# ipfs/go-libp2p-pubsub

Hardware: AMD Instinct MI355X
Metric: deliveries/sec (peer×msg) at 1M peers, 1/2/4/8 GPU; % of HBM roofline (higher is better)
Workload: dtype u64

## Files before the change

go-libp2p-pubsub_amd/csrc/api.cpp:

```cpp
#include <algorithm>
#include <cstdio>
#include <cstdlib>
#include <cstring>

#include "engine.hpp"
#include "psengine_plan.h"

using namespace psamd;

namespace {

TopicHost* join_topic(ps_engine* e, uint32_t topic) {
  if (!topic_ok(e, topic)) {
    e->fail(PS_E_STATE, "no such topic");
    return nullptr;
  }
  TopicHost& T = e->topics[topic];
  if (T.kind != Kind::Join) {
    e->fail(PS_E_STATE, "topic topology was set explicitly");
    return nullptr;
  }
  return &T;
}

// ... 99 lines not shown
  g_abi_error = buf;
  return PS_E_INVAL;
}

static bool env_flag(const char* name, bool cur) {
  const char* v = std::getenv(name);
  return v ? std::atoi(v) != 0 : cur;
}
static uint32_t env_u32(const char* name, int lo, int hi, uint32_t cur) {
  const char* v = std::getenv(name);
  return v ? static_cast<uint32_t>(std::min(hi, std::max(lo, std::atoi(v)))) : cur;
}
static uint64_t env_u64(const char* name, int base, uint64_t cur) {
  const char* v = std::getenv(name);
  return v ? std::strtoull(v, nullptr, base) : cur;
}

static void read_switches(ps_engine* e) {
  constexpr int kAny = 0x7FFFFFFF;
  auto& s = e->env;
  auto& d = e->drain.env;
  s.host_timing = env_flag("PSAMD_HOST_TIMING", s.host_timing);
  s.flood_profile = env_flag("PSAMD_FLOOD_PROFILE", s.flood_profile);
  if (const char* v = std::getenv("PSAMD_CHAIN_PROFILE")) s.chain_prof_path = v;
  d.timing = env_flag("PSAMD_DRAIN_TIMING", d.timing);
  if (!env_flag("PSAMD_AB", false)) return;
  d.slab_ids = std::max<uint64_t>(kDrainSegBits, env_u64("PSAMD_DRAIN_SLAB_IDS", 10, d.slab_ids));
  if (const char* v = std::getenv("PSAMD_DRAIN_EMIT")) d.staged = std::strcmp(v, "direct") != 0;
  if (const char* v = std::getenv("PSAMD_DRAIN_ASYNC_OUT")) d.mapped_out = std::strcmp(v, "mapped") == 0;
  if (const char* v = std::getenv("PSAMD_DRAIN_SHARED")) d.share = std::strcmp(v, "private") != 0;
  if (const char* v = std::getenv("PSAMD_LOAD_COUNT")) d.load_rows = std::strcmp(v, "rows") == 0;
  s.twin = env_flag("PSAMD_TWIN", s.twin);
  s.expand_opts = env_flag("PSAMD_NARROW", true) ? 0u : kExpandNoNarrow;
  s.chain_words_lead = env_u32("PSAMD_CHAIN_WORDS_LEAD", 0, 1 << 20, s.chain_words_lead);
  s.upload_reuse = env_flag("PSAMD_UPLOAD_REUSE", s.upload_reuse);
  s.sig_windows = env_flag("PSAMD_SIG_WINDOWS", s.sig_windows);
  s.fuse_reduce = env_flag("PSAMD_FUSE_REDUCE", s.fuse_reduce);
  ps_plan_opts o = e->opts;
  o.gpu_build = env_flag("PSAMD_GPU_BUILD", o.gpu_build);
  o.flood = env_flag("PSAMD_FLOOD", o.flood);
  if (!env_flag("PSAMD_PULL_PAIR", true)) o.chain_max = o.chain_max_groups = 1;
  if (const char* v = std::getenv("PSAMD_XCHG_OVERLAP")) o.xchg_overlap = std::atoi(v) != 0;
  o.chain_max = env_u32("PSAMD_CHAIN", 1, kChainLevels, o.chain_max);
  o.chain_max_groups = env_u32("PSAMD_CHAIN", 1, kChainLevels, o.chain_max_groups);
  o.overlap = env_flag("PSAMD_OVERLAP", o.overlap);
  o.overlap_min_rounds = env_u32("PSAMD_OVERLAP_ROUNDS", 2, kAny, o.overlap_min_rounds);
  o.overlap_min_bytes = env_u64("PSAMD_OVERLAP_BYTES", 10, o.overlap_min_bytes);
  o.pad_words = env_u32("PSAMD_PAD_WORDS", 2, kAny, o.pad_words);
  o.chain_tail = env_flag("PSAMD_CHAIN_TAIL", o.chain_tail);
  if (const char* v = std::getenv("PSAMD_LAUNCH_BYTES"))
    o.launch_bytes = static_cast<uint64_t>(std::max(0.0, std::atof(v)));
  o.chain_words = env_u32("PSAMD_CHAIN_WORDS", 256, 1 << 20, o.chain_words);
  o.flood_words = env_u32("PSAMD_FLOOD_WORDS", 64, 1 << 16, o.flood_words);
  o.flood_spin_ticks = static_cast<uint32_t>(env_u64("PSAMD_FLOOD_SPIN_TICKS", 0, o.flood_spin_ticks));
  o.flood_top_bytes = env_u64("PSAMD_FLOOD_TOP_BYTES", 0, o.flood_top_bytes);
  o.flood_min_rounds = env_u32("PSAMD_FLOOD_MIN_ROUNDS", 1, kAny, o.flood_min_rounds);
  o.chain_waves = env_u32("PSAMD_CHAIN_WAVES", 0, 16, o.chain_waves);
  if (!check_opts(o)) e->opts = o;
}

int ps_plan_opts_default(ps_plan_opts* out) {
  if (!out) return PS_E_INVAL;
  *out = default_plan_opts();
  return PS_OK;
}

// ... 861 lines not shown
```

go-libp2p-pubsub_amd/csrc/engine.hpp:

```cpp
#pragma once
#include <hip/hip_runtime.h>

#include <chrono>
#include <cstdlib>
#include <cstdint>
#include <map>
#include <memory>
#include <string>
#include <utility>
#include <vector>

#include "dist.hpp"
#include "kernels.hpp"
#include "psengine.h"
#include "tree.hpp"

namespace psamd {

constexpr uint32_t kMaxRoundsCap = 4096;
constexpr uint32_t kAlignedRowsMax = 2 * (PS_MAX_ROUNDS + 1);
constexpr uint32_t kMaxStartRound = 200;
constexpr uint32_t kDefaultWindow = 65536;
constexpr uint32_t kMaxWindow = 1u << 30;

// ... 767 lines not shown
  return t < e->last_pos.size() && !e->last_pos[t].empty() ? e->last_pos[t].data() : nullptr;
}
inline uint32_t window_bit(const uint32_t* bits, uint32_t li) { return bits ? bits[li] : li; }
inline const std::vector<uint32_t>& peer_node_map(ps_engine* e, uint32_t topic, const TopicDev& d) {
  auto& pm = e->peer_node[topic];
  if (e->peer_node_epoch.size() != e->topics.size()) e->peer_node_epoch.assign(e->topics.size(), ~0ull);
  if (e->peer_node_epoch[topic] != e->graph_epoch) {
    pm.assign(e->cfg.n_peers, kNone);
    const uint32_t u0 = (d.flags & kTopicRootLocal) ? 1 : 0;
    for (uint32_t k = u0; k < d.n_nodes; ++k) pm[e->node_peer[d.nbase + k]] = k;
    e->peer_node_epoch[topic] = e->graph_epoch;
  }
  return pm;
}

int plan_window_layout(ps_engine* e, const std::vector<RunMsg>& msgs, const std::vector<WinSlice>& win,
                       WindowLayout& L);
bool plan_pull_chunks(ps_engine* e, const WindowLayout& L);
bool plan_pair_chunks(ps_engine* e, const WindowLayout& L, uint32_t first);
bool plan_flood_tasks(ps_engine* e, const WindowLayout& L, uint32_t rounds);
int plan_ghost(ps_engine* e, const WindowLayout& L, bool* changed);
void annotate_chunks(ps_engine* e, const WindowLayout& L);
uint32_t plan_flood_rounds(const ps_engine* e, const WindowLayout& L);
bool deep_window(const ps_engine* e, const WindowLayout& L);
int plan_window_schedule(ps_engine* e, const std::vector<RunMsg>& msgs, const std::vector<WinSlice>& win,
                         WindowLayout& L, WindowSchedule& S);
void plan_schedule_pairs(ps_engine* e, const WindowLayout& L, WindowSchedule& S);
uint32_t round_grid(const ps_engine* e, const WindowLayout& L, const WindowSchedule& S, uint32_t r);

int run_body(ps_engine* e, ps_stats* st, bool may_defer);
bool accumulate_window(ps_stats* st, const uint64_t* hs, const uint64_t* ha, uint32_t r, uint32_t planned0,
                       uint32_t mode, uint32_t flood_rounds, uint32_t launches, int32_t world,
                       const std::vector<uint8_t>& kinds, bool by_round = true);
bool split_aligned_window(ps_stats* st, const uint64_t* hs, uint32_t r, uint32_t true_rounds,
                          const AlignedSplit& sp, std::string* why = nullptr);

}
```

go-libp2p-pubsub_amd/csrc/kernels.hip:

```cpp
#include <algorithm>

#include "devutil.hpp"
#include "kernels.hpp"

namespace psamd {

namespace {

using namespace dev;

__device__ __forceinline__ uint32_t wave_incl_scan(uint32_t v) {
  const int lane = threadIdx.x & 63;
#pragma unroll
  for (int d = 1; d < 64; d <<= 1) {
    uint32_t t = __shfl_up(v, d, 64);
    if (lane >= d) v += t;
  }
  return v;
}

__device__ __forceinline__ uint32_t block_excl_scan(uint32_t v, uint32_t* total) {
  __shared__ uint32_t wsum[kBlock / 64];
  const int lane = threadIdx.x & 63, wid = threadIdx.x >> 6;
  uint32_t inc = wave_incl_scan(v);
// ... 223 lines not shown
        const int q = __ffsll(static_cast<long long>(b)) - 1;
        rec[q] = hop_round(round);
        b &= b - 1;
      }
    }
  }
}

__device__ __forceinline__ void mark_next(const ExpandArgs& a, uint32_t c) {
  a.next_flag[c] = 1;
  a.blk_flag[c >> kFlagBlockShift] = 1;
}

__device__ __forceinline__ uint32_t rl(uint32_t v, uint32_t lane) {
  return static_cast<uint32_t>(__builtin_amdgcn_readlane(static_cast<int>(v), static_cast<int>(lane)));
}

__device__ __forceinline__ uint32_t pow2_shift(uint32_t W) { return 32u - __clz(W - 1u); }

#define PSAMD_LDS_DMA(g, lds_base, N)                                            \
  __builtin_amdgcn_global_load_lds((const __attribute__((address_space(1))) void*)(g), \
                                   (__attribute__((address_space(3))) void*)(lds_base), N, 0, 0)

constexpr uint32_t kStageWords = 704;
constexpr uint32_t kStageBytes = 512;
struct __attribute__((aligned(16))) WaveStage {
  uint64_t words[kStageWords];
  uint8_t flags[kStageBytes];
  uint8_t gens[kStageBytes];
};

struct EntryCtr {
  uint32_t ent = 0, ent_words = 0, kids = 0, mesh_kids = 0, clear = 0;
};

__device__ __forceinline__ bool ext_rows(const ExpandArgs& a, uint32_t W, uint32_t tflags) {
  return a.ext_cur != nullptr && W >= 64 && W <= kStageWords && !(tflags & (kTopicSingleStart | kTopicMesh));
}
constexpr uint32_t ext_whole(uint32_t W) { return W << 16; }
__device__ __forceinline__ uint32_t ext_of(const ExpandArgs& a, uint32_t p, uint32_t W) {
  const uint32_t x = a.ext_cur[p];
  return (x >> 16) <= W && (x & 0xFFFFu) <= (x >> 16) ? x : ext_whole(W);
}

template <bool kRecord>
__device__ void expand_direct(const ExpandArgs& a, uint32_t p, uint32_t rs, uint32_t deg,
                              uint32_t c0, uint32_t W, uint32_t nbase, uint32_t tflags,
                              uint64_t wbase, uint32_t lane, uint32_t cur, uint32_t round,
                              ExpandCtr& k, EntryCtr& ec) {
  const bool mesh = (tflags & kTopicMesh) != 0;
  const bool split = (tflags & kEntrySplit) != 0;
  const bool listed = mesh || split;
  const bool is_root = p == nbase && (tflags & kTopicRootLocal);
  const bool single = (tflags & kTopicSingleStart) && !mesh;
  const uint64_t* src = (single && !is_root) ? a.seen : a.a_cur;
  const uint64_t pw = wbase + static_cast<uint64_t>(p - nbase) * W;
  const uint64_t cbase = wbase - static_cast<uint64_t>(nbase) * W;
  const bool ext = ext_rows(a, W, tflags);
  const uint32_t xe = ext && !is_root ? ext_of(a, p, W) : ext_whole(W);
  const uint32_t xlo = xe & 0xFFFFu, xhi = xe >> 16;
  ec.ent += 1;
  ec.ent_words += W;
  ec.kids += deg;
  if (mesh) ec.mesh_kids += deg;
  for (uint32_t j0 = 0; j0 < deg; j0 += 64) {
    const uint32_t cd = min(64u, deg - j0);
    uint32_t cj = 0, fj = 0, gj = 0;
    if (lane < cd) {
      cj = listed ? a.col[rs + j0 + lane] : c0 + j0 + lane;
      if (!(cj & kRemoteBit)) {
        fj = a.node_flags[cj];
        gj = mesh ? 0u : a.gen[cj];
      }
    }
    if (split) {
      for (uint32_t jj = 0; jj < cd; ++jj) {
        const uint32_t c = rl(cj, jj);
        if (!(c & kRemoteBit)) continue;
        const uint32_t dest = (c >> kRemoteRankShift) & 0xFu;
        uint8_t* region = a.send + a.send_off[dest];
        uint32_t base = 0;
        if (lane == 0) base = atomicAdd(reinterpret_cast<uint32_t*>(region), W);
        base = static_cast<uint32_t>(__shfl(static_cast<int>(base), 0, 64));
        XItem* out = reinterpret_cast<XItem*>(region + kRegionHeader) + base;
        for (uint32_t w = lane; w < W; w += 64) {
          XItem it;
          it.node = c & kRemoteIdMask;
          it.word = w;
          it.mask = src[pw + w];
          out[w] = it;
        }
      }
    }
    if (W >= 64) {
      for (uint32_t wb = 0; wb < W; wb += 64) {
        const uint32_t w = wb + lane;
        const bool active = w < W;
        const uint64_t m = active && w >= xlo && w < xhi ? src[pw + w] : 0ull;
        for (uint32_t jj = 0; jj < cd; ++jj) {
          const uint32_t f = rl(fj, jj);
          if (!(f & kNodeLive)) continue;
          const uint32_t c = rl(cj, jj);
          const bool stale = !mesh && rl(gj, jj) != cur;
          const bool internal = (f & kNodeInternal) != 0;
          uint64_t nm = 0;
          if (active)
            nm = deliver_word<kRecord>(a, mesh, stale, internal && !single,
                                       cbase + static_cast<uint64_t>(c) * W + w, m, round, k);
          if (internal && __ballot(nm != 0) && lane == 0) {
            mark_next(a, c);
            if (ext) a.ext_next[c] = xe;
          }
        }
      }
    } else {
      const uint32_t sh = pow2_shift(W);
      const uint32_t wp = 1u << sh;
      const uint32_t w = lane & (wp - 1u);
      const uint32_t jl = lane >> sh;
      const uint32_t groups = 64u >> sh;
      const uint64_t gmask = (wp == 64u ? ~0ull : ((1ull << wp) - 1ull)) << (jl << sh);
      const uint64_t m = w < W ? src[pw + w] : 0ull;
      for (uint32_t jb = 0; jb < cd; jb += groups) {
        const uint32_t jj = jb + jl;
        const uint32_t c = static_cast<uint32_t>(__shfl(static_cast<int>(cj), static_cast<int>(jj), 64));
        const uint32_t f = static_cast<uint32_t>(__shfl(static_cast<int>(fj), static_cast<int>(jj), 64));
        const uint32_t g = static_cast<uint32_t>(__shfl(static_cast<int>(gj), static_cast<int>(jj), 64));
        const bool live = (w < W) && (jj < cd) && (f & kNodeLive);
        uint64_t nm = 0;
        if (live)
          nm = deliver_word<kRecord>(a, mesh, !mesh && g != cur,
                                     (f & kNodeInternal) != 0 && !single,
                                     cbase + static_cast<uint64_t>(c) * W + w, m, round, k);
        const uint64_t bal = __ballot(nm != 0);
        if (live && w == 0 && (f & kNodeInternal) && (bal & gmask)) mark_next(a, c);
      }
    }
    if (!mesh && lane < cd && (fj & kNodeLive))
      a.gen[cj] = static_cast<uint8_t>(cur);
  }
  if (mesh || is_root) {
    for (uint32_t w = lane; w < W; w += 64) a.a_cur[pw + w] = 0;
    ec.clear += W;
  }
}

template <bool kRecord>
__device__ void expand_wide(const ExpandArgs& a, WaveStage& ws, uint32_t p, uint32_t deg,
                            uint32_t c0, uint32_t W, uint32_t nbase, uint32_t fl, uint64_t wbase,
                            uint32_t lane, uint32_t cur, uint32_t round, ExpandCtr& k,
                            EntryCtr& ec) {
  const bool is_root = p == nbase && (fl & kTopicRootLocal);
  const bool from_seen = (fl & kTopicSingleStart) && !is_root;
  const bool keep = !(fl & kTopicSingleStart);
  const uint64_t pw = wbase + static_cast<uint64_t>(p - nbase) * W;
  const uint64_t cbase = wbase - static_cast<uint64_t>(nbase) * W;
  const uint32_t* row = reinterpret_cast<const uint32_t*>((from_seen ? a.seen : a.a_cur) + pw);
  uint32_t fj = 0, gj = 0;
  if (lane < deg) {
    fj = a.node_flags[c0 + lane];
    gj = a.gen[c0 + lane];
  }
  ec.ent += 1;
  ec.ent_words += W;
  ec.kids += deg;
  uint64_t got = 0;
  for (uint32_t w0 = 0; w0 < W; w0 += kStageWords) {
    const uint32_t len = min(kStageWords, W - w0);
// ... 217 lines not shown
        if (e.xe) a.ext_next[c] = e.xe;
      }
    }
  }
  ec.ent += static_cast<uint32_t>(__popcll(fmask));
  ec.ent_words += static_cast<uint32_t>(wave_sum_u64(L));
  ec.kids += ktotal;
  return flat;
}

template <bool kRecord, bool kDirect>
__global__ __launch_bounds__(kBlock) __attribute__((amdgpu_waves_per_eu(6))) void k_expand(ExpandArgs a,
                                                                                            uint32_t round) {
  __shared__ WaveStage stage_lds[kDirect ? 1 : kBlock / 64];
  const uint32_t lane = threadIdx.x & 63;
  const uint32_t wave =
      __builtin_amdgcn_readfirstlane((blockIdx.x * kBlock + threadIdx.x) >> 6);
  WaveStage& ws = stage_lds[kDirect ? 0 : __builtin_amdgcn_readfirstlane(threadIdx.x >> 6)];
  const uint32_t n_waves = (gridDim.x * kBlock) >> 6;
  const uint32_t n = *a.n_front;
  const uint32_t cur = a.gen_cur & 0xFF;

  ExpandCtr k;
  EntryCtr ec;

  const uint32_t v = __builtin_amdgcn_readfirstlane(
      (gridDim.x & 7u) ? wave
                       : ((blockIdx.x & 7u) * (gridDim.x >> 3) + (blockIdx.x >> 3)) * (kBlock / 64) +
                             (threadIdx.x >> 6));
  for (uint64_t e0 = v; e0 < n; e0 += 64ull * n_waves) {
    const uint64_t el = e0 + static_cast<uint64_t>(lane) * n_waves;
    uint32_t bp = 0, brs = 0, bdeg = 0, bc0 = 0, bW = 0, bnb = 0, bfl = 0, bwl = 0, bwh = 0, bex = 0;
    uint32_t brl = 0, brh = 0, bcl = 0, bch = 0, bnd = 0, bst = 0;
    if (el < n) {
      bp = a.frontier[el];
      const uint32_t t = a.node_topic[bp];
      brs = a.row_ptr[bp];
      bdeg = a.row_ptr[bp + 1] - brs;
      const TopicDev T = a.topics[t];
      bW = T.W;
      bnb = T.nbase;
      bfl = T.flags | ((a.node_flags[bp] & kNodeSplit) ? kEntrySplit : 0u);
      bwl = static_cast<uint32_t>(T.wbase);
      bwh = static_cast<uint32_t>(T.wbase >> 32);
      if (bdeg && T.W) bc0 = a.col[brs];
      bex = ext_rows(a, T.W, T.flags) && !(bp == T.nbase && (T.flags & kTopicRootLocal)) ? ext_of(a, bp, T.W)
                                                                                          : ext_whole(T.W);
    }
    const uint32_t nb = static_cast<uint32_t>(__popcll(__ballot(el < n)));
    const bool is_root = bp == bnb && (bfl & kTopicRootLocal);
    const bool staged = el < n && bW > 0 && !(bfl & (kTopicMesh | kEntrySplit)) && bW <= kStageWords && bdeg <= 64;
    if constexpr (!kRecord && !kDirect) {
      if (flat_on(a)) {
        const bool short_row = staged && !is_root && (bex >> 16) - (bex & 0xFFFFu) < kFlatWords;
        const uint64_t wbase = (static_cast<uint64_t>(bwh) << 32) | bwl;
        const uint64_t src = reinterpret_cast<uint64_t>(((bfl & kTopicSingleStart) ? a.seen : a.a_cur) + wbase +
                                                        static_cast<uint64_t>(bp - bnb) * bW + (bex & 0xFFFFu));
        const uint64_t crow = wbase + static_cast<uint64_t>(bc0 - bnb) * bW;
        if (expand_flat(a, ws, short_row, bW, bex, short_row && ext_rows(a, bW, bfl), bdeg, bc0, src, crow,
                        !(bfl & kTopicSingleStart), lane, cur, k, ec))
          bW = 0;
      }
    }
    if (el < n && bW) {
      const uint64_t wbase = (static_cast<uint64_t>(bwh) << 32) | bwl;
      const bool from_seen = (bfl & kTopicSingleStart) && !is_root;
      const uint64_t rp = reinterpret_cast<uint64_t>((from_seen ? a.seen : a.a_cur) + wbase +
                                                     static_cast<uint64_t>(bp - bnb) * bW + (bex & 0xFFFFu));
      brl = static_cast<uint32_t>(rp);
      brh = static_cast<uint32_t>(rp >> 32);
      const uint64_t cb = wbase + static_cast<uint64_t>(bc0 - bnb) * bW;
      bcl = static_cast<uint32_t>(cb);
      bch = static_cast<uint32_t>(cb >> 32);
      bnd = ((bc0 + bdeg + 3u) >> 2) - (bc0 >> 2);
      const uint32_t Ls = (bex >> 16) - (bex & 0xFFFFu);
      bst = staged ? (Ls + (Ls & 1u)) | (4u * bnd) << 16 : ~0u;
    }
    uint32_t q = 0;
    while (q < nb) {
      const uint32_t W0 = rl(bW, q), d0 = rl(bdeg, q), f0 = rl(bfl, q);
      if (W0 == 0) {
        ++q;
        continue;
      }
      const bool direct = (f0 & (kTopicMesh | kEntrySplit)) || d0 > 64;
      if (direct || kDirect) {
        if (direct && kDirect)
          expand_direct<kRecord>(a, rl(bp, q), rl(brs, q), d0, rl(bc0, q), W0, rl(bnb, q), f0,
                                 (static_cast<uint64_t>(rl(bwh, q)) << 32) | rl(bwl, q), lane,
                                 cur, round, k, ec);
        ++q;
        continue;
      }
      if (W0 > kStageWords) {
        expand_wide<kRecord>(a, ws, rl(bp, q), d0, rl(bc0, q), W0, rl(bnb, q), f0,
                                     (static_cast<uint64_t>(rl(bwh, q)) << 32) | rl(bwl, q), lane,
                                     cur, round, k, ec);
        ++q;
        continue;
// ... 16 lines not shown
          const uint32_t c0 = rl(bc0, i);
          const uint32_t xe = rl(bex, i), lo = xe & 0xFFFFu, L = (xe >> 16) - lo;
          const uint32_t* row =
              reinterpret_cast<const uint32_t*>((static_cast<uint64_t>(rl(brh, i)) << 32) | rl(brl, i));
          uint32_t* dst = reinterpret_cast<uint32_t*>(ws.words + off);
          if ((W & 1u) == 0) {
            for (uint32_t d = 0; d < 2 * L; d += 256)
              if (d + 4 * lane < 2 * L) PSAMD_LDS_DMA(row + d + 4 * lane, dst + d, 16);
          } else {
            for (uint32_t d = 0; d < 2 * L; d += 64)
              if (d + lane < 2 * L) PSAMD_LDS_DMA(row + d + lane, dst + d, 4);
          }
          const uint32_t nd = rl(bnd, i);
          if (lane < nd) {
            PSAMD_LDS_DMA(reinterpret_cast<const uint32_t*>(a.node_flags) + (c0 >> 2) + lane,
                          ws.flags + doff, 4);
            PSAMD_LDS_DMA(reinterpret_cast<const uint32_t*>(a.gen) + (c0 >> 2) + lane,
                          ws.gens + doff, 4);
          }
          off += L + (L & 1u);
          doff += 4u * nd;
        }
        asm volatile("s_waitcnt vmcnt(0)" ::: "memory");
      }
      {
        uint32_t off = 0, doff = 0;
        for (uint32_t i = q; i < q + nq; ++i) {
          const uint32_t W = rl(bW, i), deg = rl(bdeg, i);
          if (W == 0) continue;
          const uint32_t c0 = rl(bc0, i);
          const uint64_t crow0 = (static_cast<uint64_t>(rl(bch, i)) << 32) | rl(bcl, i);
          const uint32_t nd = rl(bnd, i);
          const uint32_t fo = doff + (c0 & 3u);
          const bool keep = !(rl(bfl, i) & kTopicSingleStart);
          const uint32_t xe = rl(bex, i), lo = xe & 0xFFFFu, hi = xe >> 16;
          ec.ent += 1;
          ec.ent_words += hi - lo;
          ec.kids += deg;
          if (W >= 64) {
            const bool ext = ext_rows(a, W, rl(bfl, i));
            uint32_t tlo = lo, thi = hi;
            if (ext) {
              tlo = hi;
              thi = lo;
              for (uint32_t wb = lo; wb < hi; wb += 64) {
                const uint32_t w = wb + lane;
                const uint64_t nz = __ballot(w < hi && ws.words[off + w - lo] != 0);
                if (nz) {
                  tlo = min(tlo, wb + static_cast<uint32_t>(__ffsll(static_cast<long long>(nz))) - 1u);
                  thi = wb + 64u - static_cast<uint32_t>(__clzll(static_cast<long long>(nz)));
                }
              }
              if (tlo >= thi) {
                tlo = thi = lo;
              } else {
                tlo &= ~1u;
                thi = (thi + 1u) & ~1u;
              }
            }
            for (uint32_t jj = 0; jj < deg; ++jj) {
              const uint32_t f = ws.flags[fo + jj];
              if (!(f & kNodeLive)) continue;
              const bool stale = ws.gens[fo + jj] != cur;
              const bool internal = (f & kNodeInternal) != 0;
              const bool store = internal && keep;
              const uint32_t c = c0 + jj;
              const uint64_t row = crow0 + static_cast<uint64_t>(jj) * W;
              bool any = false;
              if (stale) {
                for (uint32_t wb = 0; wb < W; wb += 128) {
                  const uint32_t w = wb + 2 * lane;
                  if (w < W) {
                    const bool in = w >= tlo && w < thi;
                    const uint4 v = in ? *reinterpret_cast<const uint4*>(ws.words + off + w - lo)
                                       : make_uint4(0u, 0u, 0u, 0u);
                    deliver_fresh2<kRecord>(a, store && (in || !ext), row + w, v, round, k);
                    any |= (v.x | v.y | v.z | v.w) != 0;
                  }
                }
              } else {
                for (uint32_t wb = tlo; wb < thi; wb += 64) {
                  const uint32_t w = wb + lane;
                  if (w < thi) {
                    const uint64_t nm = deliver_tree<kRecord>(a, store, row + w, ws.words[off + w - lo], round, k);
                    any |= nm != 0;
                  }
                }
              }
              if (internal && __ballot(any) && lane == 0) {
                mark_next(a, c);
                if (ext) a.ext_next[c] = tlo | thi << 16;
              }
            }
          } else {
            const uint32_t sh = pow2_shift(W);
            const uint32_t wp = 1u << sh;
            const uint32_t w = lane & (wp - 1u);
            const uint32_t jl = lane >> sh;
            const uint32_t groups = 64u >> sh;
            const uint64_t gmask = (wp == 64u ? ~0ull : ((1ull << wp) - 1ull)) << (jl << sh);
            const uint64_t m = w < W ? ws.words[off + w] : 0ull;
            for (uint32_t jb = 0; jb < deg; jb += groups) {
              const uint32_t jj = jb + jl;
              const bool valid = (w < W) && (jj < deg);
              const uint32_t f = valid ? ws.flags[fo + jj] : 0u;
              const bool live = valid && (f & kNodeLive);
              const bool stale = ws.gens[fo + jj] != cur;
              const uint32_t c = c0 + jj;
              const uint64_t cw = crow0 + static_cast<uint64_t>(jj) * W + w;
              uint64_t nm = 0;
              if (__ballot(live && !stale) == 0) {
                if (live) {
                  deliver_fresh<kRecord>(a, keep && (f & kNodeInternal), cw, m, round, k);
                  nm = m;
                }
              } else if (live) {
                if (stale) {
                  deliver_fresh<kRecord>(a, keep && (f & kNodeInternal), cw, m, round, k);
                  nm = m;
                } else {
                  nm = deliver_tree<kRecord>(a, keep && (f & kNodeInternal), cw, m, round, k);
                }
              }
              const uint64_t bal = __ballot(nm != 0);
              if (live && w == 0 && (f & kNodeInternal) && (bal & gmask)) mark_next(a, c);
            }
          }
          if (lane < deg && (ws.flags[fo + lane] & kNodeLive))
            a.gen[c0 + lane] = static_cast<uint8_t>(cur);
          if (rl(bp, i) == rl(bnb, i) && (rl(bfl, i) & kTopicRootLocal)) {
            const uint64_t pw = (static_cast<uint64_t>(rl(bwh, i)) << 32) | rl(bwl, i);
            for (uint32_t w = lane; w < W; w += 64) a.a_cur[pw + w] = 0;
            ec.clear += W;
          }
          off += (hi - lo) + ((hi - lo) & 1u);
          doff += 4u * nd;
        }
      }
      q += nq;
    }
  }

  const uint64_t s_deliv = wave_sum_u64(k.deliv);
  const uint64_t s_dup = wave_sum_u64(k.dup);
  const uint64_t s_sr = wave_sum_u64(k.sr);
  const uint64_t s_sw = wave_sum_u64(k.sw);
  const uint64_t s_aw = wave_sum_u64(k.aw);
  if (lane == 0) {
    uint64_t* out = a.partials + static_cast<uint64_t>(wave) * kNumCtr;
    out[kCtrDeliveries] = s_deliv;
    out[kCtrDuplicates] = s_dup;
    out[kCtrEntries] = ec.ent;
    out[kCtrEntryWords] = ec.ent_words;
    out[kCtrChildren] = ec.kids;
    out[kCtrMeshChildren] = ec.mesh_kids;
    out[kCtrSeenReads] = s_sr;
    out[kCtrSeenWrites] = s_sw;
    out[kCtrArrivalWrites] = s_aw;
    out[kCtrClearWords] = ec.clear;
  }
}

__global__ __launch_bounds__(kBlock) void k_stage_copy(StageCopy c) {
  const uint32_t tid = blockIdx.x * kBlock + threadIdx.x, nth = gridDim.x * kBlock;
  for (uint32_t k = 0; k < c.n; ++k)
    for (uint32_t i = tid; i < c.words[k]; i += nth) c.dst[k][i] = c.src[k][i];
}

template <bool kRecord>
__global__ __launch_bounds__(kBlock) void k_apply(ApplyArgs a, uint32_t round) {
  const uint64_t total = a.cap_pre[a.world];
  uint64_t deliv = 0, dup = 0;
  for (uint64_t i = static_cast<uint64_t>(blockIdx.x) * kBlock + threadIdx.x; i < total;
       i += static_cast<uint64_t>(gridDim.x) * kBlock) {
    uint32_t src = 0;
    while (i >= a.cap_pre[src + 1]) ++src;
    const uint8_t* region = a.recv + a.recv_off[src];
    const uint64_t k = i - a.cap_pre[src];
    if (k >= *reinterpret_cast<const uint32_t*>(region)) continue;
    const XItem it = reinterpret_cast<const XItem*>(region + kRegionHeader)[k];
    const uint8_t f = a.node_flags[it.node];
    if (!(f & kNodeLive) || it.mask == 0) {
      if ((f & kNodeLive) && (f & kNodeInternal)) {
        const TopicDev T = a.topics[a.node_topic[it.node]];
        if (!(T.flags & kTopicSingleStart))
// ... 479 lines not shown
```

go-libp2p-pubsub_amd/csrc/kernels.hpp:

```cpp
#pragma once
#include <hip/hip_runtime.h>

#include <cstdint>

namespace psamd {

enum : uint8_t {
  kNodeLive = 1,
  kNodeInternal = 2,
  kNodeSplit = 4,
};

constexpr uint32_t kRemoteBit = 0x80000000u;
constexpr uint32_t kRemoteRankShift = 27;
constexpr uint32_t kRemoteIdMask = (1u << kRemoteRankShift) - 1u;
constexpr int kMaxRanks = 16;

struct XItem {
  uint32_t node;
  uint32_t word;
  uint64_t mask;
};
constexpr uint32_t kRegionHeader = 16;

// ... 43 lines not shown
  kCtrChildren,
  kCtrMeshChildren,
  kCtrSeenReads,
  kCtrSeenWrites,
  kCtrArrivalWrites,
  kCtrClearWords,
  kNumCtr
};

struct ExpandArgs {
  const uint32_t* frontier;
  const uint32_t* n_front;
  const uint32_t* row_ptr;
  const uint32_t* col;
  const uint16_t* node_topic;
  const uint8_t* node_flags;
  const TopicDev* topics;
  uint64_t* a_cur;
  uint64_t* a_next;
  uint64_t* seen;
  uint32_t* ext_cur;
  uint32_t* ext_next;
  uint8_t* gen;
  uint8_t* next_flag;
  uint8_t* blk_flag;
  uint64_t* partials;
  uint16_t* hop_rec;
  uint32_t gen_cur;
  uint8_t* send;
  uint64_t send_off[kMaxRanks];
  uint32_t opts;
};
constexpr uint32_t kExpandNoNarrow = 1;

struct PullChunk {
  uint32_t node_begin, node_end;
  uint32_t topic;
  uint32_t p_lo, p_hi;
  uint32_t W;
  uint32_t row0_lo, row0_hi;
  uint32_t e_lo, e_hi;
  uint32_t c_lo, c_hi;
  uint32_t gin, gout;
  uint32_t group;
  uint32_t lvl0;
};
constexpr uint32_t kPullMaxKids = 512;
constexpr uint32_t kNoneNode = 0xFFFFFFFFu;
constexpr uint32_t kPullWords = 1024;

struct ShipEntry {
  uint32_t node;
  uint32_t dst;
};
struct GhostSeg {
  uint64_t rbase[kMaxRanks];
  uint64_t sbase[kMaxRanks];
  uint32_t rw;
  uint32_t topic;
  uint32_t flags;
  uint32_t gbase[kMaxRanks];
};
constexpr uint32_t kSegInPlace = 1u;
struct RankRows {
  const uint64_t* seen;
  const uint8_t* gen;
// ... 670 lines not shown
```

go-libp2p-pubsub_amd/csrc/run.cpp:

```cpp
#include <algorithm>
#include <chrono>
#include <atomic>
#include <cstdio>
#include <cstdlib>
#include <cstring>
#include <thread>

#include "engine.hpp"
#include "gbuild.hpp"

namespace {
inline void cpu_relax() {
#if defined(__x86_64__) || defined(__i386__)
  __builtin_ia32_pause();
#else
  std::this_thread::yield();
#endif
}
}

namespace psamd {

namespace {

// ... 962 lines not shown
    std::string xerr;
    hipError_t xe =
        e->transport->exchange(a.send, s_off, s_len, e->d_recv.as<uint8_t>(), r_off, r_len, s, &xerr);
    if (xe != hipSuccess) return e->fail(PS_E_DEVICE, xerr);
    st->xchg_path = PS_XCHG_COPY;
    st->xchg_rounds += 1;
    for (const uint64_t n : r_len) st->xchg_bytes += n;
    HIP_TRY(launch_apply(apply_args(rr), rr, record, s), "apply");
    return PS_OK;
  }

  int grow_stats_rows(uint32_t planned) {
    const uint32_t rows = std::min<uint32_t>(L.round_cap, std::max(planned + 1, 2 * stats_rows));
    DevBuf grown;
    HIP_TRY(grown.ensure(static_cast<size_t>(rows + 1) * kNumCtr * 8), "grow stats");
    HIP_TRY(hipMemcpyAsync(grown.p, e->d_stats.p, static_cast<size_t>(stats_rows + 1) * kNumCtr * 8,
                           hipMemcpyDeviceToDevice, s),
            "keep stats");
    HIP_TRY(hipStreamSynchronize(s), "sync");
    std::swap(grown.p, e->d_stats.p);
    std::swap(grown.bytes, e->d_stats.bytes);
    stats = e->d_stats.as<uint64_t>();
    stats_rows = rows;
    return PS_OK;
  }

  int compaction_rounds() {
    const int32_t world = e->world;
    uint32_t planned = L.planned0;
    if (world > 1)
      for (auto* v : {&s_off, &s_len, &r_off, &r_len}) v->assign(world, 0);
    uint32_t* ext[2] = {nullptr, nullptr};
    if (world == 1) {
      HIP_TRY(e->d_ext0.ensure(static_cast<size_t>(e->n_pad) * 4), "alloc extents");
      HIP_TRY(e->d_ext1.ensure(static_cast<size_t>(e->n_pad) * 4), "alloc extents");
      ext[0] = e->d_ext0.as<uint32_t>();
      ext[1] = e->d_ext1.as<uint32_t>();
    }
    HIP_TRY(seed_round(0, arr[0]), "seed");
    HIP_TRY(compact_frontier(0, 0), "compact");
    while (true) {
      for (; r < planned && r < L.round_cap;) {
        ++r;
        a.a_cur = arr[(r - 1) & 1];
        a.a_next = arr[r & 1];
        a.ext_cur = ext[(r - 1) & 1];
        a.ext_next = ext[r & 1];
        const bool xr = layout_regions(r);
        if (xr)
          for (int32_t q = 0; q < world; ++q)
            if (s_len[q]) HIP_TRY(hipMemsetAsync(a.send + s_off[q], 0, kRegionHeader, s), "reset header");
        HIP_TRY(time_mark(true), "event");
        ++launches;
        const uint32_t grid_r = r <= L.planned0 ? round_grid(e, L, S, r) : e->expand_grid;
        a.partials = partials;
        HIP_TRY(launch_expand(a, r, record, grid_r, s), "expand");
        uint32_t waves_r = grid_r * (kBlock / 64);
        if (L.need_direct) {
          a.partials = partials + static_cast<size_t>(waves_r) * kNumCtr;
          HIP_TRY(launch_expand_direct(a, r, record, e->expand_grid, s), "expand direct");
          waves_r += n_waves;
        }
        HIP_TRY(time_mark(false), "event");
        if (xr)
          if (const int rc = exchange_apply(r)) return rc;
        HIP_TRY(seed_round(r, a.a_next), "seed");
        HIP_TRY(compact_frontier(r, waves_r), "compact");
      }
// ... 93 lines not shown
        }
      }
    }
    return PS_OK;
  }

  int finish_blocking() {
    const uint32_t planned0 = L.planned0;
    HIP_TRY(hipEventSynchronize(e->ev_run1), "sync");
    const auto t_sync = Clock::now();
    const ps_stats keep = *st;
    float ms = 0.f;
    HIP_TRY(hipEventElapsedTime(&ms, e->ev_run0, e->ev_run1), "elapsed");
    st->run_ms += ms;
    for (size_t i = 0; i < ev_used; i += 2) {
      float k = 0.f;
      HIP_TRY(hipEventElapsedTime(&k, e->ev_k[i], e->ev_k[i + 1]), "elapsed");
      st->expand_ms += k;
      const size_t q = ev_round[i / 2];
      if (q < PS_MAX_ROUNDS) st->expand_ms_per_round[q] += k;
    }
    std::vector<uint64_t> hs(static_cast<size_t>(r + 1 + S.reach_rows) * kNumCtr), ha;
    HIP_TRY(hipMemcpyAsync(hs.data(), stats, hs.size() * 8, hipMemcpyDeviceToHost, s), "read stats");
    if (e->world > 1) {
      ha.resize(static_cast<size_t>(planned0 + 1) * kNumCtr);
      HIP_TRY(hipMemcpyAsync(ha.data(), e->d_apply_stats.p, ha.size() * 8, hipMemcpyDeviceToHost, s),
              "read apply stats");
    }
    HIP_TRY(hipStreamSynchronize(s), "sync");
    if (S.mode == PS_MODE_FLOOD && e->env.flood_profile && e->flood_prof_waves) flood_profile_report(e);
    if (cprof) chain_profile_dump(e, planned0);
    if (std::string why; L.aligned && !split_aligned_window(st, hs.data(), r, L.true_rounds, L.split, &why))
      return e->fail(PS_E_DEVICE, "level-aligned window: reach counts disagree with the per-level counters (" + why + ")");
    if (!accumulate_window(st, hs.data(), ha.data(), r, planned0, S.mode, S.flood_rounds, launches, e->world,
                           e->round_kind, !L.aligned)) {
      e->flood_broken = true;
      *st = keep;
      if (e->env.host_timing) std::fprintf(stderr, "[psengine] k_flood timed out: window re-run per round\n");
      return run_window(e, msgs, win, st);
    }
    if (e->env.host_timing) {
      char tail[80];
      std::snprintf(tail, sizeof tail, ", wait %.3f ms, tail %.3f ms",
                    std::chrono::duration<double, std::milli>(t_sync - t_enq).count(),
                    std::chrono::duration<double, std::milli>(Clock::now() - t_sync).count());
      host_timing_line("window", tail);
    }
    if (record)
      if (const int rc = read_hop_record()) return rc;
    remember_window();
    return PS_OK;
  }

  int run() {
    int rc;
    if ((rc = window_layout())) return rc;
    if (L.wtot == 0 && e->world == 1) return PS_OK;
    t_w1 = Clock::now();
    if ((rc = ensure_window_buffers())) return rc;
    if ((rc = plan_window_schedule(e, msgs, win, L, S))) return rc;
    if ((rc = upload_window_plans()) || (rc = ensure_schedule_buffers())) return rc;
    t_w3 = Clock::now();
    if ((rc = upload_reach_pieces())) return rc;
    if ((rc = choose_streams()) || (rc = start_window())) return rc;
    if ((rc = L.level ? level_rounds() : compaction_rounds())) return rc;
    const bool defer = defers(r);
// ... 2 lines not shown
    t_enq = Clock::now();
    return defer ? finish_deferred() : finish_blocking();
  }
};

int run_window(ps_engine* e, const std::vector<RunMsg>& msgs, const std::vector<WinSlice>& win, ps_stats* st) {
  return WindowRun{e, msgs, win, st}.run();
}

int run_phase(ps_engine* e, const std::vector<RunMsg>& msgs, const std::vector<WinSlice>& per, ps_stats* st) {
  const uint32_t nt = static_cast<uint32_t>(e->topics.size());
  const uint32_t cap = e->cfg.msg_window;
  uint32_t n_win = 0;
  for (const auto& v : per) n_win = std::max(n_win, (v.n + cap - 1) / cap);
  std::vector<WinSlice> win(nt);
  for (uint32_t k = 0; k < n_win; ++k) {
    for (uint32_t t = 0; t < nt; ++t) {
      const uint32_t lo = k * cap;
      win[t].idx = per[t].idx + std::min(lo, per[t].n);
      win[t].n = lo < per[t].n ? std::min(cap, per[t].n - lo) : 0;
    }
    e->defer_last = e->defer_phase && k + 1 == n_win;
    const uint64_t seq0 = e->window_seq;
    int rc = run_window(e, msgs, win, st);
    e->defer_last = false;
    if (!rc && e->window_seq != seq0 && !(rc = sink_window(e)) && !(rc = load_window(e)) && !(rc = hops_window(e)) &&
        !(rc = downstream_window(e)) && !(rc = cut_window(e)))
      rc = report_window(e);
    if (rc) return rc;
  }
  return PS_OK;
}

}

bool accumulate_window(ps_stats* st, const uint64_t* hs, const uint64_t* ha, uint32_t r, uint32_t planned0,
                       uint32_t mode, uint32_t flood_rounds, uint32_t launches, int32_t world,
                       const std::vector<uint8_t>& kinds, bool by_round) {
  const bool pull = mode == PS_MODE_LEVEL_PULL || mode == PS_MODE_FLOOD;
  std::memset(st->round_kernel, 0, sizeof(st->round_kernel));
  for (uint32_t q = 1; q <= r; ++q) {
    const uint8_t kind = q < kinds.size() ? kinds[q] : static_cast<uint8_t>(pull ? PS_K_PULL : PS_K_EXPAND);
    const uint64_t* c = &hs[static_cast<size_t>(q) * kNumCtr];
    const uint64_t app_d = (world > 1 && q <= planned0) ? ha[static_cast<size_t>(q) * kNumCtr + kCtrDeliveries] : 0;
    const uint64_t app_u = (world > 1 && q <= planned0) ? ha[static_cast<size_t>(q) * kNumCtr + kCtrDuplicates] : 0;
    st->deliveries += c[kCtrDeliveries] + app_d;
    st->duplicates += c[kCtrDuplicates] + app_u;
    st->frontier_entries += c[kCtrEntries];
    st->child_visits += c[kCtrChildren];
    st->edge_words += c[kCtrSeenWrites];
    uint64_t b;
    if (pull)
      b = c[kCtrChildren] * (kind == PS_K_FLOOD ? 7 : (kind == PS_K_PAIR2 || kind == PS_K_CHAIN2) ? 5 : 6) +
          c[kCtrMeshChildren] * 1 +
          c[kCtrEntryWords] * 8 + c[kCtrSeenWrites] * 8;
    else
      b = c[kCtrEntries] * 18 + c[kCtrEntryWords] * 8 + c[kCtrClearWords] * 8 + c[kCtrChildren] * 3 +
          c[kCtrMeshChildren] * 4 + c[kCtrSeenReads] * 8 + c[kCtrSeenWrites] * 8 + c[kCtrArrivalWrites] * 8;
    st->expand_bytes += b;
    if (q < PS_MAX_ROUNDS) {
      st->round_kernel[q] = kind;
      st->expand_bytes_per_round[q] += b;
      if (by_round) {
        st->deliveries_per_round[q] += c[kCtrDeliveries] + app_d;
        st->frontier_per_round[q] += static_cast<uint32_t>(c[kCtrEntries]);
      }
// ... 275 lines not shown
  }
  if (f.deferred && f.signalled) {
    const volatile uint64_t* flag = f.sig;
    const auto t0 = std::chrono::steady_clock::now();
    for (uint64_t spin = 0; *flag != f.seq; ++spin) {
      cpu_relax();
      if ((spin & 255) == 255) {
        const hipError_t q = hipStreamQuery(f.stream ? f.stream : e->stream);
        if (q != hipSuccess && q != hipErrorNotReady) return e->fail(PS_E_DEVICE, "window: stream failed");
        if (q == hipSuccess && *flag != f.seq) return e->fail(PS_E_DEVICE, "window: completion flag missing");
        const auto us =
            std::chrono::duration_cast<std::chrono::microseconds>(std::chrono::steady_clock::now() - t0).count();
        if (us > 2000)
          std::this_thread::sleep_for(std::chrono::microseconds(20));
        else if (us > 50)
          std::this_thread::yield();
      }
    }
    std::atomic_thread_fence(std::memory_order_acquire);
    const volatile uint64_t* t = f.sig;
    f.st.run_ms += static_cast<double>(t[2] - t[1]) * 1e-5;
  } else if (f.deferred) {
    HIP_TRY(hipEventSynchronize(f.ev1), "sync");
    float ms = 0.f;
    HIP_TRY(hipEventElapsedTime(&ms, f.ev0, f.ev1), "elapsed");
    f.st.run_ms += ms;
  }
  if (f.deferred) {
    f.deferred = false;
    const bool aligned = f.split.n_segs > 0;
    if (std::string why; aligned && !split_aligned_window(&f.st, f.hs, f.r, f.true_rounds, f.split, &why))
      return e->fail(PS_E_DEVICE, "level-aligned window: reach counts disagree with the per-level counters (" + why +
                                      ")");
    if (!accumulate_window(&f.st, f.hs, f.ha, f.r, f.planned0, f.mode, f.flood_rounds, f.launches, f.world,
                           f.kinds, !aligned)) {
      e->flood_broken = true;
      return e->fail(PS_E_DEVICE, "k_flood: a dependency wait timed out (waves not co-resident?); "
                                  "per-round launches from now on");
    }
  }
  if (out) *out = f.st;
  return PS_OK;
}

}
```

Measured before the change: 40310 billion.

## Read frontier rows from seen bitmap via arrival extents instead of a_cur

In the expand kernel, extent-tracked rows are now read directly from the seen bitmap rather than the separate a_cur frontier copy. Each expanded child records its arrival extent in ext_next, and internal nodes skip writing a_cur. Extent tracking is also extended to rows narrower than 64 words, and loads are restricted to the extent window. The aim is to cut the extra per-word frontier writes and reads, at the cost of extent bookkeeping, clearing ext_cur per entry, and a new device error flag the host checks.

```diff
diff --git a/go-libp2p-pubsub_amd/csrc/api.cpp b/go-libp2p-pubsub_amd/csrc/api.cpp
--- a/go-libp2p-pubsub_amd/csrc/api.cpp
+++ b/go-libp2p-pubsub_amd/csrc/api.cpp
@@ -155,6 +155,7 @@
   if (const char* v = std::getenv("PSAMD_LOAD_COUNT")) d.load_rows = std::strcmp(v, "rows") == 0;
   s.twin = env_flag("PSAMD_TWIN", s.twin);
   s.expand_opts = env_flag("PSAMD_NARROW", true) ? 0u : kExpandNoNarrow;
+  if (!env_flag("PSAMD_EXPAND_ALIAS", true)) s.expand_opts |= kExpandNoAlias;
   s.chain_words_lead = env_u32("PSAMD_CHAIN_WORDS_LEAD", 0, 1 << 20, s.chain_words_lead);
   s.upload_reuse = env_flag("PSAMD_UPLOAD_REUSE", s.upload_reuse);
   s.sig_windows = env_flag("PSAMD_SIG_WINDOWS", s.sig_windows);
diff --git a/go-libp2p-pubsub_amd/csrc/engine.hpp b/go-libp2p-pubsub_amd/csrc/engine.hpp
--- a/go-libp2p-pubsub_amd/csrc/engine.hpp
+++ b/go-libp2p-pubsub_amd/csrc/engine.hpp
@@ -823,6 +823,7 @@
 bool accumulate_window(ps_stats* st, const uint64_t* hs, const uint64_t* ha, uint32_t r, uint32_t planned0,
                        uint32_t mode, uint32_t flood_rounds, uint32_t launches, int32_t world,
                        const std::vector<uint8_t>& kinds, bool by_round = true);
+bool expand_extent_error(const uint64_t* hs, uint32_t r, uint32_t mode);
 bool split_aligned_window(ps_stats* st, const uint64_t* hs, uint32_t r, uint32_t true_rounds,
                           const AlignedSplit& sp, std::string* why = nullptr);
 
diff --git a/go-libp2p-pubsub_amd/csrc/kernels.hip b/go-libp2p-pubsub_amd/csrc/kernels.hip
--- a/go-libp2p-pubsub_amd/csrc/kernels.hip
+++ b/go-libp2p-pubsub_amd/csrc/kernels.hip
@@ -279,15 +279,40 @@
 
 struct EntryCtr {
   uint32_t ent = 0, ent_words = 0, kids = 0, mesh_kids = 0, clear = 0;
+  uint32_t bad = 0;
 };
 
+__device__ __forceinline__ bool alias_on(const ExpandArgs& a) { return (a.opts & kExpandNoAlias) == 0; }
 __device__ __forceinline__ bool ext_rows(const ExpandArgs& a, uint32_t W, uint32_t tflags) {
-  return a.ext_cur != nullptr && W >= 64 && W <= kStageWords && !(tflags & (kTopicSingleStart | kTopicMesh));
+  return a.ext_cur != nullptr && (W >= 64 || alias_on(a)) && W <= kStageWords &&
+         !(tflags & (kTopicSingleStart | kTopicMesh));
+}
+__device__ __forceinline__ bool alias_rows(const ExpandArgs& a, uint32_t W, uint32_t tflags) {
+  return alias_on(a) && ext_rows(a, W, tflags);
 }
 constexpr uint32_t ext_whole(uint32_t W) { return W << 16; }
-__device__ __forceinline__ uint32_t ext_of(const ExpandArgs& a, uint32_t p, uint32_t W) {
+__device__ __forceinline__ uint32_t ext_of(const ExpandArgs& a, uint32_t p, uint32_t W, bool* bad) {
   const uint32_t x = a.ext_cur[p];
-  return (x >> 16) <= W && (x & 0xFFFFu) <= (x >> 16) ? x : ext_whole(W);
+  const uint32_t lo = x & 0xFFFFu, hi = x >> 16;
+  if (alias_on(a)) {
+    *bad = !(lo < hi && hi <= W && ((lo | hi) & 1u) == 0);
+    return *bad ? 0u : x;
+  }
+  return hi <= W && lo <= hi ? x : ext_whole(W);
+}
+__device__ __forceinline__ void ext_fold(uint64_t nz, uint32_t wb, uint32_t& tlo, uint32_t& thi) {
+  if (nz) {
+    tlo = min(tlo, wb + static_cast<uint32_t>(__ffsll(static_cast<long long>(nz))) - 1u);
+    thi = wb + 64u - static_cast<uint32_t>(__clzll(static_cast<long long>(nz)));
+  }
+}
+__device__ __forceinline__ void ext_close(uint32_t lo, uint32_t& tlo, uint32_t& thi) {
+  if (tlo >= thi) {
+    tlo = thi = lo;
+  } else {
+    tlo &= ~1u;
+    thi = (thi + 1u) & ~1u;
+  }
 }
 
 template <bool kRecord>
@@ -300,11 +325,27 @@
   const bool listed = mesh || split;
   const bool is_root = p == nbase && (tflags & kTopicRootLocal);
   const bool single = (tflags & kTopicSingleStart) && !mesh;
-  const uint64_t* src = (single && !is_root) ? a.seen : a.a_cur;
+  const bool ext = ext_rows(a, W, tflags);
+  const bool alias = ext && alias_on(a);
+  const uint64_t* src = ((single || alias) && !is_root) ? a.seen : a.a_cur;
   const uint64_t pw = wbase + static_cast<uint64_t>(p - nbase) * W;
   const uint64_t cbase = wbase - static_cast<uint64_t>(nbase) * W;
-  const bool ext = ext_rows(a, W, tflags);
-  const uint32_t xe = ext && !is_root ? ext_of(a, p, W) : ext_whole(W);
+  uint32_t xe = ext_whole(W);
+  if (ext && !is_root) {
+    bool bad = false;
+    xe = ext_of(a, p, W, &bad);
+    if (alias) a.ext_cur[p] = 0;
+    if (bad) {
+      ec.bad = 1;
+      return;
+    }
+  } else if (alias) {
+    uint32_t tlo = W, thi = 0;
+    for (uint32_t wb = 0; wb < W; wb += 64)
+      ext_fold(__ballot(wb + lane < W && src[pw + wb + lane] != 0), wb, tlo, thi);
+    ext_close(0, tlo, thi);
+    xe = tlo | thi << 16;
+  }
   const uint32_t xlo = xe & 0xFFFFu, xhi = xe >> 16;
   ec.ent += 1;
   ec.ent_words += W;
@@ -352,7 +393,7 @@
           const bool internal = (f & kNodeInternal) != 0;
           uint64_t nm = 0;
           if (active)
-            nm = deliver_word<kRecord>(a, mesh, stale, internal && !single,
+            nm = deliver_word<kRecord>(a, mesh, stale, internal && !single && !alias,
                                        cbase + static_cast<uint64_t>(c) * W + w, m, round, k);
           if (internal && __ballot(nm != 0) && lane == 0) {
             mark_next(a, c);
@@ -367,7 +408,7 @@
       const uint32_t jl = lane >> sh;
       const uint32_t groups = 64u >> sh;
       const uint64_t gmask = (wp == 64u ? ~0ull : ((1ull << wp) - 1ull)) << (jl << sh);
-      const uint64_t m = w < W ? src[pw + w] : 0ull;
+      const uint64_t m = w < W && w >= xlo && w < xhi ? src[pw + w] : 0ull;
       for (uint32_t jb = 0; jb < cd; jb += groups) {
         const uint32_t jj = jb + jl;
         const uint32_t c = static_cast<uint32_t>(__shfl(static_cast<int>(cj), static_cast<int>(jj), 64));
@@ -377,10 +418,13 @@
         uint64_t nm = 0;
         if (live)
           nm = deliver_word<kRecord>(a, mesh, !mesh && g != cur,
-                                     (f & kNodeInternal) != 0 && !single,
+                                     (f & kNodeInternal) != 0 && !single && !alias,
                                      cbase + static_cast<uint64_t>(c) * W + w, m, round, k);
         const uint64_t bal = __ballot(nm != 0);
-        if (live && w == 0 && (f & kNodeInternal) && (bal & gmask)) mark_next(a, c);
+        if (live && w == 0 && (f & kNodeInternal) && (bal & gmask)) {
+          mark_next(a, c);
+          if (ext) a.ext_next[c] = xe;
+        }
       }
     }
     if (!mesh && lane < cd && (fj & kNodeLive))
@@ -664,6 +708,7 @@
     const uint64_t el = e0 + static_cast<uint64_t>(lane) * n_waves;
     uint32_t bp = 0, brs = 0, bdeg = 0, bc0 = 0, bW = 0, bnb = 0, bfl = 0, bwl = 0, bwh = 0, bex = 0;
     uint32_t brl = 0, brh = 0, bcl = 0, bch = 0, bnd = 0, bst = 0;
+    bool xbad = false;
     if (el < n) {
       bp = a.frontier[el];
       const uint32_t t = a.node_topic[bp];
@@ -676,9 +721,18 @@
       bwl = static_cast<uint32_t>(T.wbase);
       bwh = static_cast<uint32_t>(T.wbase >> 32);
       if (bdeg && T.W) bc0 = a.col[brs];
-      bex = ext_rows(a, T.W, T.flags) && !(bp == T.nbase && (T.flags & kTopicRootLocal)) ? ext_of(a, bp, T.W)
-                                                                                          : ext_whole(T.W);
-    }
+      bex = ext_whole(T.W);
+      if (T.W && ext_rows(a, T.W, T.flags) && !(bp == T.nbase && (T.flags & kTopicRootLocal))) {
+        bool bad = false;
+        bex = ext_of(a, bp, T.W, &bad);
+        if (!kDirect && bdeg <= 64 && alias_on(a)) {
+          a.ext_cur[bp] = 0;
+          xbad = bad;
+          if (bad) bW = 0;
+        }
+      }
+    }
+    if (__ballot(xbad)) ec.bad = 1;
     const uint32_t nb = static_cast<uint32_t>(__popcll(__ballot(el < n)));
     const bool is_root = bp == bnb && (bfl & kTopicRootLocal);
     const bool staged = el < n && bW > 0 && !(bfl & (kTopicMesh | kEntrySplit)) && bW <= kStageWords && bdeg <= 64;
@@ -686,17 +740,18 @@
       if (flat_on(a)) {
         const bool short_row = staged && !is_root && (bex >> 16) - (bex & 0xFFFFu) < kFlatWords;
         const uint64_t wbase = (static_cast<uint64_t>(bwh) << 32) | bwl;
-        const uint64_t src = reinterpret_cast<uint64_t>(((bfl & kTopicSingleStart) ? a.seen : a.a_cur) + wbase +
+        const bool in_seen = (bfl & kTopicSingleStart) || alias_rows(a, bW, bfl);
+        const uint64_t src = reinterpret_cast<uint64_t>((in_seen ? a.seen : a.a_cur) + wbase +
                                                         static_cast<uint64_t>(bp - bnb) * bW + (bex & 0xFFFFu));
         const uint64_t crow = wbase + static_cast<uint64_t>(bc0 - bnb) * bW;
         if (expand_flat(a, ws, short_row, bW, bex, short_row && ext_rows(a, bW, bfl), bdeg, bc0, src, crow,
-                        !(bfl & kTopicSingleStart), lane, cur, k, ec))
+                        !in_seen, lane, cur, k, ec))
           bW = 0;
       }
     }
     if (el < n && bW) {
       const uint64_t wbase = (static_cast<uint64_t>(bwh) << 32) | bwl;
-      const bool from_seen = (bfl & kTopicSingleStart) && !is_root;
+      const bool from_seen = ((bfl & kTopicSingleStart) || alias_rows(a, bW, bfl)) && !is_root;
       const uint64_t rp = reinterpret_cast<uint64_t>((from_seen ? a.seen : a.a_cur) + wbase +
                                                      static_cast<uint64_t>(bp - bnb) * bW + (bex & 0xFFFFu));
       brl = static_cast<uint32_t>(rp);
@@ -779,31 +834,22 @@
           const uint64_t crow0 = (static_cast<uint64_t>(rl(bch, i)) << 32) | rl(bcl, i);
           const uint32_t nd = rl(bnd, i);
           const uint32_t fo = doff + (c0 & 3u);
-          const bool keep = !(rl(bfl, i) & kTopicSingleStart);
+          const bool ext = ext_rows(a, W, rl(bfl, i));
+          const bool keep = !(rl(bfl, i) & kTopicSingleStart) && !(ext && alias_on(a));
           const uint32_t xe = rl(bex, i), lo = xe & 0xFFFFu, hi = xe >> 16;
           ec.ent += 1;
           ec.ent_words += hi - lo;
           ec.kids += deg;
           if (W >= 64) {
-            const bool ext = ext_rows(a, W, rl(bfl, i));
             uint32_t tlo = lo, thi = hi;
             if (ext) {
               tlo = hi;
               thi = lo;
               for (uint32_t wb = lo; wb < hi; wb += 64) {
                 const uint32_t w = wb + lane;
-                const uint64_t nz = __ballot(w < hi && ws.words[off + w - lo] != 0);
-                if (nz) {
-                  tlo = min(tlo, wb + static_cast<uint32_t>(__ffsll(static_cast<long long>(nz))) - 1u);
-                  thi = wb + 64u - static_cast<uint32_t>(__clzll(static_cast<long long>(nz)));
-                }
+                ext_fold(__ballot(w < hi && ws.words[off + w - lo] != 0), wb, tlo, thi);
               }
-              if (tlo >= thi) {
-                tlo = thi = lo;
-              } else {
-                tlo &= ~1u;
-                thi = (thi + 1u) & ~1u;
-              }
+              ext_close(lo, tlo, thi);
             }
             for (uint32_t jj = 0; jj < deg; ++jj) {
               const uint32_t f = ws.flags[fo + jj];
@@ -846,7 +892,14 @@
             const uint32_t jl = lane >> sh;
             const uint32_t groups = 64u >> sh;
             const uint64_t gmask = (wp == 64u ? ~0ull : ((1ull << wp) - 1ull)) << (jl << sh);
-            const uint64_t m = w < W ? ws.words[off + w] : 0ull;
+            const uint64_t m = w >= lo && w < hi ? ws.words[off + w - lo] : 0ull;
+            uint32_t xn = 0;
+            if (ext) {
+              uint32_t tlo = hi, thi = lo;
+              ext_fold(__ballot(lane < W && m != 0), 0, tlo, thi);
+              ext_close(lo, tlo, thi);
+              xn = tlo | thi << 16;
+            }
             for (uint32_t jb = 0; jb < deg; jb += groups) {
               const uint32_t jj = jb + jl;
               const bool valid = (w < W) && (jj < deg);
@@ -870,7 +923,10 @@
                 }
               }
               const uint64_t bal = __ballot(nm != 0);
-              if (live && w == 0 && (f & kNodeInternal) && (bal & gmask)) mark_next(a, c);
+              if (live && w == 0 && (f & kNodeInternal) && (bal & gmask)) {
+                mark_next(a, c);
+                if (ext) a.ext_next[c] = xn;
+              }
             }
           }
           if (lane < deg && (ws.flags[fo + lane] & kNodeLive))
@@ -897,7 +953,7 @@
     uint64_t* out = a.partials + static_cast<uint64_t>(wave) * kNumCtr;
     out[kCtrDeliveries] = s_deliv;
     out[kCtrDuplicates] = s_dup;
-    out[kCtrEntries] = ec.ent;
+    out[kCtrEntries] = ec.ent | static_cast<uint64_t>(ec.bad) << kCtrEntriesErrShift;
     out[kCtrEntryWords] = ec.ent_words;
     out[kCtrChildren] = ec.kids;
     out[kCtrMeshChildren] = ec.mesh_kids;
diff --git a/go-libp2p-pubsub_amd/csrc/kernels.hpp b/go-libp2p-pubsub_amd/csrc/kernels.hpp
--- a/go-libp2p-pubsub_amd/csrc/kernels.hpp
+++ b/go-libp2p-pubsub_amd/csrc/kernels.hpp
@@ -99,6 +99,8 @@
   uint32_t opts;
 };
 constexpr uint32_t kExpandNoNarrow = 1;
+constexpr uint32_t kExpandNoAlias = 2;
+constexpr uint32_t kCtrEntriesErrShift = 40;
 
 struct PullChunk {
   uint32_t node_begin, node_end;
diff --git a/go-libp2p-pubsub_amd/csrc/run.cpp b/go-libp2p-pubsub_amd/csrc/run.cpp
--- a/go-libp2p-pubsub_amd/csrc/run.cpp
+++ b/go-libp2p-pubsub_amd/csrc/run.cpp
@@ -1018,8 +1018,11 @@
       for (auto* v : {&s_off, &s_len, &r_off, &r_len}) v->assign(world, 0);
     uint32_t* ext[2] = {nullptr, nullptr};
     if (world == 1) {
-      HIP_TRY(e->d_ext0.ensure(static_cast<size_t>(e->n_pad) * 4), "alloc extents");
-      HIP_TRY(e->d_ext1.ensure(static_cast<size_t>(e->n_pad) * 4), "alloc extents");
+      for (DevBuf* b : {&e->d_ext0, &e->d_ext1}) {
+        bool fresh = false;
+        HIP_TRY(b->ensure(static_cast<size_t>(e->n_pad) * 4, &fresh), "alloc extents");
+        if (fresh) HIP_TRY(hipMemsetAsync(b->p, 0, b->bytes, s), "clear extents");
+      }
       ext[0] = e->d_ext0.as<uint32_t>();
       ext[1] = e->d_ext1.as<uint32_t>();
     }
@@ -1179,6 +1182,8 @@
     if (cprof) chain_profile_dump(e, planned0);
     if (std::string why; L.aligned && !split_aligned_window(st, hs.data(), r, L.true_rounds, L.split, &why))
       return e->fail(PS_E_DEVICE, "level-aligned window: reach counts disagree with the per-level counters (" + why + ")");
+    if (expand_extent_error(hs.data(), r, S.mode))
+      return e->fail(PS_E_DEVICE, "k_expand: a frontier entry without a valid arrival extent");
     if (!accumulate_window(st, hs.data(), ha.data(), r, planned0, S.mode, S.flood_rounds, launches, e->world,
                            e->round_kind, !L.aligned)) {
       e->flood_broken = true;
@@ -1247,6 +1252,13 @@
   return PS_OK;
 }
 
+}
+
+bool expand_extent_error(const uint64_t* hs, uint32_t r, uint32_t mode) {
+  if (mode != PS_MODE_COMPACT) return false;
+  for (uint32_t q = 1; q <= r; ++q)
+    if (hs[static_cast<size_t>(q) * kNumCtr + kCtrEntries] >> kCtrEntriesErrShift) return true;
+  return false;
 }
 
 bool accumulate_window(ps_stats* st, const uint64_t* hs, const uint64_t* ha, uint32_t r, uint32_t planned0,
@@ -1588,6 +1600,8 @@
     if (std::string why; aligned && !split_aligned_window(&f.st, f.hs, f.r, f.true_rounds, f.split, &why))
       return e->fail(PS_E_DEVICE, "level-aligned window: reach counts disagree with the per-level counters (" + why +
                                       ")");
+    if (expand_extent_error(f.hs, f.r, f.mode))
+      return e->fail(PS_E_DEVICE, "k_expand: a frontier entry without a valid arrival extent");
     if (!accumulate_window(&f.st, f.hs, f.ha, f.r, f.planned0, f.mode, f.flood_rounds, f.launches, f.world,
                            f.kinds, !aligned)) {
       e->flood_broken = true;
```

Measured after the change: 40240 billion. No clear change (-0.2%).
